# microsoft/foldingdiff

Hardware: AMD Instinct MI355X
Metric: backbones/sec (L=128, T=1000, bs=512) (higher is better)
Workload: dtype f32 (fp16 hi/lo split operands, 3x v_mfma_f32_{32x32x16,16x16x32}_f16 per product, fp32 accumulate)

## Files before the change

### foldingdiff_amd/csrc/ffn16.hip

```cpp
#include <cstdlib>
#include <type_traits>

#include "fdmi_kernels.h"
#include "img_common.h"

namespace fdmi {
namespace ffn {

typedef float f32x4 __attribute__((ext_vector_type(4)));
typedef const __attribute__((address_space(3))) u32x4* lds_cu128_t;
__device__ __forceinline__ unsigned lds_addr(const void* p) { return (unsigned)(unsigned long long)(lds_ptr_t)(const_cast<void*>(p)); }
__device__ __forceinline__ u32x4 lds_u128(unsigned a) { return *(lds_cu128_t)(unsigned long long)a; }
__device__ __forceinline__ f16x8 lds_f16x8(unsigned a) { return __builtin_bit_cast(f16x8, lds_u128(a)); }

__device__ __forceinline__ void swap16(unsigned& vdst, unsigned& src) {
  const auto r = __builtin_amdgcn_permlane16_swap(vdst, src, false, false);
  vdst = r[0];
  src = r[1];
}
__device__ __forceinline__ float quad_sum(float x) {
  unsigned a = __builtin_bit_cast(unsigned, x), b = a;
  swap32(a, b);
  float m = __builtin_bit_cast(float, a) + __builtin_bit_cast(float, b);
  a = __builtin_bit_cast(unsigned, m);
  b = a;
  swap16(a, b);
  return __builtin_bit_cast(float, a) + __builtin_bit_cast(float, b);
}

template <int V> using IC = std::integral_constant<int, V>;
template <int LO, int HI, class F>
__device__ __forceinline__ void static_for(F&& f) {
  if constexpr (LO < HI) {
    f(IC<LO>{});
    static_for<LO + 1, HI>(f);
  }
}

#ifndef FDMI_FFN_DBG
#define FDMI_FFN_DBG 0
#endif
#ifndef FDMI_FFN_ST_AUX
#define FDMI_FFN_ST_AUX 0
#endif
#ifndef FDMI_FFN_PRIO
#define FDMI_FFN_PRIO 2
#endif

__device__ __forceinline__ f32x4 mfma16(const f16x8& a, const f16x8& b, const f32x4& c) {
  return __builtin_amdgcn_mfma_f32_16x16x32_f16(a, b, c, 0, 0, 0);
}

constexpr int NW = 8;
constexpr int TILE = 2048;
constexpr int STEP = 4 * TILE;
constexpr int SPS = 2;
constexpr int STAGE = SPS * STEP;
constexpr int NST = 3;
constexpr int PPW = STAGE / 1024 / NW;
constexpr int OFF_W = 0;
constexpr int OFF_X = NST * STAGE;
__host__ __device__ constexpr int off_p(int nkt) { return OFF_X + NW * nkt * 1024; }

template <int NKT, bool TAIL, bool PROF>
__global__ __launch_bounds__(64 * NW) void ffn16_kernel(FfnArgs p) {
  static_assert(NKT == 12 || NKT == 6, "d_model 384 or 192, intermediate size 2 d_model");
  constexpr int D = 32 * NKT;
  constexpr int NG = NKT;
  constexpr int SPG = 2 * NKT;
  constexpr int STG = SPG / SPS;
  static_assert(STG % NST == 0, "a group is a whole number of ring turns: its first stage always sits in slot 0");
  constexpr int NSA = TAIL ? NKT * NKT / 2 : 0;
  static_assert((NSA / SPS) % NST == 0 && NSA % SPS == 0, "whole ring turns");
  constexpr int W_BYTES = (NSA / SPS + NG * STG) * STAGE;
  constexpr int OFF_P = off_p(NKT);
  constexpr int OFF_P1 = OFF_P + 5 * D * 4;
  extern __shared__ __attribute__((aligned(16))) unsigned char smem[];
  const int tid = threadIdx.x, lane = tid & 63;
  const int wq = __builtin_amdgcn_readfirstlane(tid >> 6);
  const int grp = wq >> 2;
  unsigned smem0 = __builtin_amdgcn_readfirstlane(lds_addr(smem));
  asm volatile("" : "+s"(smem0));
  auto lane_id = [&]() __attribute__((always_inline)) {
    int ln;
    asm volatile("v_mbcnt_lo_u32_b32 %0, -1, 0\n\tv_mbcnt_hi_u32_b32 %0, -1, %0" : "=v"(ln));
    return ln;
  };
  auto lane_off_of = [](int ln) __attribute__((always_inline)) { return (unsigned)((ln >> 4) * 256 + (ln & 15) * 16); };

  {
    float* par = reinterpret_cast<float*>(smem + OFF_P);
    for (int i = tid; i < 2 * D; i += 64 * NW) par[i] = p.bi[i];
    for (int i = tid; i < D; i += 64 * NW) {
      par[2 * D + i] = p.bd[i];
      par[3 * D + i] = p.gamma[i];
      par[4 * D + i] = p.beta[i] * p.out_scale;
      if constexpr (TAIL) {
        par[5 * D + i] = p.bo[i] * (1.0f / p.ao_scale);
        par[6 * D + i] = p.g1[i];
        par[7 * D + i] = p.b1[i] * p.a_scale;
      }
    }
  }

  int w_src = 0, w_slot = 0;
  const __amdgpu_buffer_rsrc_t rs_w = __builtin_amdgcn_make_buffer_rsrc(const_cast<unsigned char*>(p.wimg), 0, W_BYTES, 0x00020000);
  auto issue_w = [&]() __attribute__((always_inline)) {
    const lds_ptr_t dst = (lds_ptr_t)(unsigned long long)(smem0 + OFF_W + (unsigned)__builtin_amdgcn_readfirstlane(w_slot));
    const int so = __builtin_amdgcn_readfirstlane(w_src);
    const int vo = lane_id() * 16;
#pragma unroll
    for (int k = 0; k < PPW; ++k) dma16(rs_w, dst + (wq + NW * k) * 1024, vo, so + (wq + NW * k) * 1024);
    w_src = w_src + STAGE == W_BYTES ? 0 : w_src + STAGE;
    w_slot = w_slot + STAGE == NST * STAGE ? 0 : w_slot + STAGE;
  };

  f16x8 ah[NKT];
  const __amdgpu_buffer_rsrc_t rs_a =
      __builtin_amdgcn_make_buffer_rsrc(const_cast<unsigned char*>(TAIL ? p.cimg : p.aimg), 0, p.a_bytes, 0x00020000);
  const __amdgpu_buffer_rsrc_t rs_h = __builtin_amdgcn_make_buffer_rsrc(const_cast<unsigned char*>(TAIL ? p.hres : p.aimg), 0, p.a_bytes, 0x00020000);
  auto row_off = [&](int r0) __attribute__((always_inline)) {
    const int ln = lane_id();
    const int row = r0 + 16 * wq + (ln & 15);
    return (unsigned)(((row >> 5) * (NKT * 256) + (row & 31)) * 16 + (ln >> 4) * 512);
  };
  u32x4 tl[NKT];
  auto load_hi = [&](int r0) __attribute__((always_inline)) {
    const unsigned hoff = row_off(r0);
#pragma unroll
    for (int kt = 0; kt < NKT; ++kt)
      ah[kt] = __builtin_bit_cast(f16x8, __builtin_amdgcn_raw_buffer_load_b128(rs_a, (int)hoff, kt * 8 * 512, 0));
  };
  auto load_lo = [&](auto KT, unsigned hoff) __attribute__((always_inline)) {
    constexpr int kt = decltype(KT)::value;
    tl[kt] = __builtin_bit_cast(u32x4, __builtin_amdgcn_raw_buffer_load_b128(rs_a, (int)hoff, (kt * 8 + 4) * 512, 0));
  };
  auto commit_lo = [&]() __attribute__((always_inline)) {
    const unsigned ax = smem0 + OFF_X + (unsigned)(wq * NKT * 1024 + lane_id() * 16);
#pragma unroll
    for (int kt = 0; kt < NKT; ++kt) *(__attribute__((address_space(3))) u32x4*)(unsigned long long)(ax + (unsigned)(kt * 1024)) = tl[kt];
  };
  const __amdgpu_buffer_rsrc_t rs_o = __builtin_amdgcn_make_buffer_rsrc(p.out, 0, p.out_bytes, 0x00020000);
  auto load_res = [&](auto KT, unsigned hoff, f32x4 (&Yr)[2 * NKT]) __attribute__((always_inline)) {
    constexpr int kt = decltype(KT)::value;
    Yr[2 * kt] = __builtin_bit_cast(f32x4, __builtin_amdgcn_raw_buffer_load_b128(rs_h, (int)hoff, kt * 8 * 512, 0));
    Yr[2 * kt + 1] = __builtin_bit_cast(f32x4, __builtin_amdgcn_raw_buffer_load_b128(rs_h, (int)hoff, (kt * 8 + 4) * 512, 0));
  };

  const bool rec = PROF && blockIdx.x == 0 && p.stamps != nullptr;
  unsigned long long* stp = PROF ? p.stamps + (size_t)wq * 16 * 16 : nullptr;
  int slot = 0;
#define FD_STAMP(i) do { if (PROF) { if (rec && slot < 16 && lane == 0) stp[slot * 16 + (i)] = __builtin_amdgcn_s_memtime(); } } while (0)
#define FD_SB() __builtin_amdgcn_sched_barrier(0)
#define FD_STAMP_G(i) do { if (PROF) { if (rec && slot == 0 && G == 1 && lane == 0) stp[15 * 16 + (i)] = __builtin_amdgcn_s_memtime(); } } while (0)

  const int n_pass = p.dims ? min(p.panels, __builtin_amdgcn_readfirstlane(p.dims[1]) >> 7) : p.panels;
  if ((int)blockIdx.x >= n_pass) return;
  const float os_up = p.up_scale, os_dn = p.down_scale, hs = 0.5f * p.g_scale;
  const f32x4 zero4 = {0.f, 0.f, 0.f, 0.f};
  f32x4 Y[2 * NKT];
  f32x4 U[4];
  f32x4 Up[4];
  u32x4 uh[2], ul[2];

  load_hi((int)blockIdx.x * 128);
  {
    const unsigned hoff = row_off((int)blockIdx.x * 128);
    static_for<0, NKT>([&](auto KT) __attribute__((always_inline)) { load_lo(KT, hoff); });
    if constexpr (TAIL) static_for<0, NKT>([&](auto KT) __attribute__((always_inline)) { load_res(KT, hoff, Y); });
  }
  issue_w();
  issue_w();
  issue_w();
  FD_WAIT_VM(3 * PPW);
  commit_lo();
  FD_WAIT_VM(2 * PPW);
  barrier_keep_vm();

  auto gelu_piece = [&](auto P, unsigned abq) __attribute__((always_inline)) {
    constexpr int pc = decltype(P)::value, pr = pc >> 2, j = pc & 3;
    const u32x2 b = *(const __attribute__((address_space(3))) u32x2*)(unsigned long long)(abq + (unsigned)((32 * pr + 2 * j) * 4));
    float o0 = __builtin_fmaf(Up[2 * pr + (j >> 1)][2 * (j & 1)], os_up, __builtin_bit_cast(float, (unsigned)b[0]));
    float o1 = __builtin_fmaf(Up[2 * pr + (j >> 1)][2 * (j & 1) + 1], os_up, __builtin_bit_cast(float, (unsigned)b[1]));
#if !(FDMI_FFN_DBG & 1)
    const float h0 = o0 * hs, h1 = o1 * hs;
    o0 = __builtin_fmaf(h0, erf_rational(o0 * 0.70710678118654752440f), h0);
    o1 = __builtin_fmaf(h1, erf_rational(o1 * 0.70710678118654752440f), h1);
#endif
    unsigned a, c;
    split_pair(o0, o1, a, c);
    uh[pr][j] = a;
    ul[pr][j] = c;
  };

  auto steps = [&](auto S0, auto S1, auto GEL, unsigned abq) __attribute__((always_inline)) {
    constexpr int s0 = decltype(S0)::value, s1 = decltype(S1)::value;
    constexpr bool gel = decltype(GEL)::value == 1, pha = decltype(GEL)::value == 2;
    auto stage_top = [&]() __attribute__((always_inline)) {
      FD_WAIT_VM(PPW);
      barrier_keep_vm();
      issue_w();
    };
    f16x8 fx[4], fy[4], xl;
    unsigned a_W, a_X;
    {
      const int ln = lane_id();
      a_W = smem0 + OFF_W + lane_off_of(ln);
      a_X = smem0 + OFF_X + (unsigned)(wq * NKT * 1024 + ln * 16);
      asm volatile("" : "+v"(a_W), "+v"(a_X));
    }
    auto plane_reads = [&](auto S, auto LO, f16x8 (&f)[4]) __attribute__((always_inline)) {
      constexpr int s = decltype(S)::value, lo = decltype(LO)::value;
      constexpr unsigned off = (unsigned)(((s / SPS) % NST) * STAGE + (s % SPS) * STEP + lo * 1024);
#if FDMI_FFN_DBG & 8
      if constexpr (lo == 1) {
#pragma unroll
        for (int t = 0; t < 4; ++t) f[t] = fx[t];
      } else
#endif
#pragma unroll
      for (int t = 0; t < 4; ++t) f[t] = lds_f16x8(a_W + off + (unsigned)(t * TILE));
      if constexpr (pha) {
        if constexpr (lo == 0 && s % (NKT / 2) == 0) xl = lds_f16x8(a_X + (unsigned)((s / (NKT / 2)) * 1024));
      } else {
        if constexpr (lo == 0 && s < NKT) xl = lds_f16x8(a_X + (unsigned)(s * 1024));
      }
    };
    auto mm = [&](auto S, auto WHICH, const f16x8 (&f)[4]) __attribute__((always_inline)) {
      constexpr int s = decltype(S)::value, which = decltype(WHICH)::value;
      if constexpr (pha) {
        constexpr int kt = s / (NKT / 2), q = s % (NKT / 2);
#pragma unroll
        for (int t = 0; t < 4; ++t) Y[4 * q + t] = mfma16(f[t], which == 1 ? xl : ah[kt], Y[4 * q + t]);
      } else if constexpr (s < NKT) {
#if !(FDMI_FFN_DBG & 4)
#pragma unroll
        for (int t = 0; t < 4; ++t) U[t] = mfma16(f[t], which == 1 ? xl : ah[s], U[t]);
#endif
      } else {
#if !(FDMI_FFN_DBG & 2)
        constexpr int pr = (s - NKT) / (NKT / 2), q = (s - NKT) % (NKT / 2);
#pragma unroll
        for (int t = 0; t < 4; ++t) Y[4 * q + t] = mfma16(f[t], __builtin_bit_cast(f16x8, which == 1 ? ul[pr] : uh[pr]), Y[4 * q + t]);
#endif
      }
    };
    plane_reads(S0, IC<0>{}, fx);
    FD_SB();
    static_for<s0, s1>([&](auto S) __attribute__((always_inline)) {
      constexpr int s = decltype(S)::value;
      constexpr bool top = s % SPS == SPS - 1;
      plane_reads(S, IC<1>{}, fy);
      FD_SB();
      if constexpr (top) {
        if (grp == 0) stage_top();
      }
#if FDMI_FFN_PRIO
      __builtin_amdgcn_s_setprio(FDMI_FFN_PRIO);
#endif
      mm(S, IC<0>{}, fx);
      mm(S, IC<1>{}, fx);
#if FDMI_FFN_PRIO
      __builtin_amdgcn_s_setprio(0);
#endif
      FD_SB();
      if constexpr (top) {
        if (grp != 0) stage_top();
      }
      if constexpr (s + 1 < s1) plane_reads(IC<s + 1>{}, IC<0>{}, fx);
      FD_SB();
      if constexpr (gel) {
        if (grp == 0) {
          static_for<0, 8>([&](auto P) __attribute__((always_inline)) {
            if constexpr (1 + decltype(P)::value * (NKT - 2) / 8 == s) gelu_piece(P, abq);
          });
        }
        FD_SB();
      }
      mm(S, IC<2>{}, fy);
      FD_SB();
      if constexpr (gel) {
        if (grp != 0) {
          static_for<0, 8>([&](auto P) __attribute__((always_inline)) {
            if constexpr (1 + decltype(P)::value * (NKT - 2) / 8 == s) gelu_piece(P, abq);
          });
        }
        FD_SB();
      }
    });
  };

  for (int panel = blockIdx.x; panel < n_pass; panel += (int)gridDim.x) {
    FD_STAMP(0);
    if constexpr (TAIL) {
      const int ln = lane_id();
      const int g = ln >> 4;
      const unsigned pb1 = smem0 + OFF_P1 + (unsigned)(8 * g * 4);
      const unsigned ax = smem0 + OFF_X + (unsigned)(wq * NKT * 1024 + ln * 16);
      {
        const float c = p.hres_inv * (1.0f / p.ao_scale);
#pragma unroll
        for (int kt = 0; kt < NKT; ++kt) {
          const u32x4 rh = __builtin_bit_cast(u32x4, Y[2 * kt]), rl = __builtin_bit_cast(u32x4, Y[2 * kt + 1]);
          const u32x4 b0 = lds_u128(pb1 + (unsigned)(kt * 128)), b1 = lds_u128(pb1 + (unsigned)(kt * 128 + 16));
#pragma unroll
          for (int j = 0; j < 2; ++j)
#pragma unroll
            for (int e = 0; e < 4; e += 2) {
              const unsigned hw = rh[2 * j + e / 2], lw = rl[2 * j + e / 2];
              const unsigned bw0 = j == 0 ? b0[e] : b1[e], bw1 = j == 0 ? b0[e + 1] : b1[e + 1];
              float v0 = fma_mix_lo(hw, c, __builtin_bit_cast(float, bw0));
              float v1 = fma_mix_hi(hw, c, __builtin_bit_cast(float, bw1));
              Y[2 * kt + j][e] = fma_mix_lo(lw, c, v0);
              Y[2 * kt + j][e + 1] = fma_mix_hi(lw, c, v1);
            }
        }
      }
      steps(IC<0>{}, IC<NSA>{}, IC<2>{}, 0u);
      const float os_ao = p.ao_scale;
      float sum = 0.f;
#pragma unroll
      for (int t = 0; t < 2 * NKT; ++t)
#pragma unroll
        for (int e = 0; e < 4; ++e) {
          Y[t][e] *= os_ao;
          sum += Y[t][e];
        }
      const float inv_n = 1.0f / (float)D;
      float mean = quad_sum(sum) * inv_n;
      asm volatile("" : "+v"(mean));
      float t2 = 0.f;
#pragma unroll
      for (int t = 0; t < 2 * NKT; ++t)
#pragma unroll
        for (int e = 0; e < 4; ++e) {
          const float dl = Y[t][e] - mean;
          Y[t][e] = dl;
          t2 = __builtin_fmaf(dl, dl, t2);
        }
      const float rstd = (1.0f / sqrtf(__builtin_fmaf(quad_sum(t2), inv_n, p.eps1))) * p.a_scale;
#pragma unroll
      for (int kt = 0; kt < NKT; ++kt) {
        const u32x4 g0 = lds_u128(pb1 + (unsigned)(D * 4 + kt * 128)), g1 = lds_u128(pb1 + (unsigned)(D * 4 + kt * 128 + 16));
        const u32x4 e0 = lds_u128(pb1 + (unsigned)(2 * D * 4 + kt * 128)), e1 = lds_u128(pb1 + (unsigned)(2 * D * 4 + kt * 128 + 16));
        float o[8];
#pragma unroll
        for (int e = 0; e < 4; ++e) {
          o[e] = __builtin_fmaf(Y[2 * kt][e] * rstd, __builtin_bit_cast(float, (unsigned)g0[e]), __builtin_bit_cast(float, (unsigned)e0[e]));
          o[4 + e] = __builtin_fmaf(Y[2 * kt + 1][e] * rstd, __builtin_bit_cast(float, (unsigned)g1[e]), __builtin_bit_cast(float, (unsigned)e1[e]));
        }
        u32x4 hv, lv;
#pragma unroll
        for (int j = 0; j < 4; ++j) {
          unsigned a, b;
          split_pair(o[2 * j], o[2 * j + 1], a, b);
          hv[j] = a;
          lv[j] = b;
        }
        ah[kt] = __builtin_bit_cast(f16x8, hv);
        *(__attribute__((address_space(3))) u32x4*)(unsigned long long)(ax + (unsigned)(kt * 1024)) = lv;
      }
    }
#pragma unroll
    for (int t = 0; t < 2 * NKT; ++t) Y[t] = zero4;
#pragma unroll
    for (int t = 0; t < 4; ++t) U[t] = zero4;
    steps(IC<0>{}, IC<NKT>{}, IC<0>{}, 0u);
    for (int G = 0; G < NG; ++G) {
#pragma unroll
      for (int t = 0; t < 4; ++t) {
        Up[t] = U[t];
        U[t] = zero4;
      }
      unsigned abq = smem0 + OFF_P + (unsigned)((64 * G + 8 * (lane_id() >> 4)) * 4);
      asm volatile("" : "+v"(abq));
      FD_STAMP_G(0);
      FD_STAMP_G(1);
      if (G + 1 < NG) {
#ifdef FDMI_FFN_NOPIPE
        static_for<0, 8>([&](auto P) __attribute__((always_inline)) { gelu_piece(P, abq); });
        steps(IC<0>{}, IC<NKT>{}, IC<0>{}, abq);
#else
        steps(IC<0>{}, IC<NKT>{}, IC<1>{}, abq);
#endif
      } else {
        static_for<0, 8>([&](auto P) __attribute__((always_inline)) { gelu_piece(P, abq); });
      }
      FD_STAMP_G(2);
      steps(IC<NKT>{}, IC<SPG>{}, IC<0>{}, 0u);
      FD_STAMP_G(3);
      if (slot == 0) FD_STAMP(1 + (G < 12 ? G : 11));
    }
    {
      const int ln = lane_id();
      const int g = ln >> 4;
      const unsigned pb = smem0 + OFF_P + (unsigned)((2 * D + 8 * g) * 4);
      const unsigned ax = smem0 + OFF_X + (unsigned)(wq * NKT * 1024 + ln * 16);
      const float ri = p.resid_inv;
      float sum = 0.f;
#pragma unroll
      for (int kt = 0; kt < NKT; ++kt) {
        const u32x4 b0 = lds_u128(pb + (unsigned)(kt * 128)), b1 = lds_u128(pb + (unsigned)(kt * 128 + 16));
        const u32x4 rh = __builtin_bit_cast(u32x4, ah[kt]), rl = lds_u128(ax + (unsigned)(kt * 1024));
#pragma unroll
        for (int j = 0; j < 2; ++j)
#pragma unroll
          for (int e = 0; e < 4; e += 2) {
            const unsigned bw0 = j == 0 ? b0[e] : b1[e], bw1 = j == 0 ? b0[e + 1] : b1[e + 1];
            float v0 = __builtin_fmaf(Y[2 * kt + j][e], os_dn, __builtin_bit_cast(float, bw0));
            float v1 = __builtin_fmaf(Y[2 * kt + j][e + 1], os_dn, __builtin_bit_cast(float, bw1));
            const unsigned hw = rh[2 * j + e / 2], lw = rl[2 * j + e / 2];
            v0 = fma_mix_lo(hw, ri, v0);
            v1 = fma_mix_hi(hw, ri, v1);
            v0 = fma_mix_lo(lw, ri, v0);
            v1 = fma_mix_hi(lw, ri, v1);
            Y[2 * kt + j][e] = v0;
            Y[2 * kt + j][e + 1] = v1;
            sum += v0;
            sum += v1;
          }
      }
      const int next = panel + (int)gridDim.x;
      load_hi(next * 128);
      const unsigned noff = row_off(next * 128);
      const float inv_n = 1.0f / (float)D;
      float mean = quad_sum(sum) * inv_n;
      asm volatile("" : "+v"(mean));
      float t2 = 0.f;
#pragma unroll
      for (int t = 0; t < 2 * NKT; ++t)
#pragma unroll
        for (int e = 0; e < 4; ++e) {
          const float dl = Y[t][e] - mean;
          Y[t][e] = dl;
          t2 = __builtin_fmaf(dl, dl, t2);
        }
      const float rstd = (1.0f / sqrtf(__builtin_fmaf(quad_sum(t2), inv_n, p.eps))) * p.out_scale;
      const unsigned ooff = row_off(panel * 128);
      static_for<0, NKT>([&](auto KT) __attribute__((always_inline)) {
        constexpr int kt = decltype(KT)::value;
        const u32x4 g0 = lds_u128(pb + (unsigned)(D * 4 + kt * 128)), g1 = lds_u128(pb + (unsigned)(D * 4 + kt * 128 + 16));
        const u32x4 e0 = lds_u128(pb + (unsigned)(2 * D * 4 + kt * 128)), e1 = lds_u128(pb + (unsigned)(2 * D * 4 + kt * 128 + 16));
        float o[8];
#pragma unroll
        for (int e = 0; e < 4; ++e) {
          o[e] = __builtin_fmaf(Y[2 * kt][e] * rstd, __builtin_bit_cast(float, (unsigned)g0[e]), __builtin_bit_cast(float, (unsigned)e0[e]));
          o[4 + e] = __builtin_fmaf(Y[2 * kt + 1][e] * rstd, __builtin_bit_cast(float, (unsigned)g1[e]), __builtin_bit_cast(float, (unsigned)e1[e]));
        }
        u32x4 hv, lv;
#pragma unroll
        for (int j = 0; j < 4; ++j) {
          unsigned a, b;
          split_pair(o[2 * j], o[2 * j + 1], a, b);
          hv[j] = a;
          lv[j] = b;
        }
#if FDMI_FFN_DBG & 16
        if (hv[0] == 0x12345678u && lv[1] == 0x9abcdef0u)
#endif
        {
          __builtin_amdgcn_raw_buffer_store_b128(hv, rs_o, (int)ooff, kt * 8 * 512, FDMI_FFN_ST_AUX);
          __builtin_amdgcn_raw_buffer_store_b128(lv, rs_o, (int)ooff, (kt * 8 + 4) * 512, FDMI_FFN_ST_AUX);
        }
        load_lo(KT, noff);
        if constexpr (TAIL) load_res(KT, noff, Y);
        FD_SB();
      });
    }
    FD_STAMP(13);
    FD_WAIT_VM(0);
    commit_lo();
    FD_STAMP(14);
    ++slot;
  }
  FD_WAIT_VM(0);
#undef FD_STAMP
#undef FD_STAMP_G
#undef FD_SB
}

static int n_cu_of(int dev) {
  static int cached[64] = {0};
  if (dev < 0 || dev >= 64) return 256;
  if (cached[dev] == 0) {
    hipDeviceProp_t prop;
    cached[dev] = (hipGetDeviceProperties(&prop, dev) == hipSuccess && prop.multiProcessorCount > 0) ? prop.multiProcessorCount : 256;
  }
  return cached[dev];
}

template <int NKT, bool TAIL>
static bool launch(const FfnArgs& p, hipStream_t s) {
  constexpr int SMEM = off_p(NKT) + (TAIL ? 8 : 5) * 32 * NKT * 4;
  static int attr_state[64] = {0};
  int dev = 0;
  (void)hipGetDevice(&dev);
  if (dev < 0 || dev >= 64) dev = 0;
  if (attr_state[dev] == 0) {
    bool ok = true;
    for (const void* f : {reinterpret_cast<const void*>(&ffn16_kernel<NKT, TAIL, false>), reinterpret_cast<const void*>(&ffn16_kernel<NKT, TAIL, true>)})
      ok = ok && hipFuncSetAttribute(f, hipFuncAttributeMaxDynamicSharedMemorySize, SMEM) == hipSuccess;
    attr_state[dev] = ok ? 1 : -1;
  }
  if (attr_state[dev] < 0) return false;
  int grid = n_cu_of(dev);
  if (grid > p.panels) grid = p.panels;
  if (grid <= 0) return true;
  if (p.stamps) hipLaunchKernelGGL((ffn16_kernel<NKT, TAIL, true>), dim3(grid), dim3(64 * NW), SMEM, s, p);
  else hipLaunchKernelGGL((ffn16_kernel<NKT, TAIL, false>), dim3(grid), dim3(64 * NW), SMEM, s, p);
  return hipGetLastError() == hipSuccess;
}

}

bool ffn16_supported(int d_model, int d_ff) { return (d_model == 384 || d_model == 192) && d_ff == 2 * d_model; }

bool launch_ffn16(const FfnArgs& p, int d_model, hipStream_t s) {
  if (p.cimg) return d_model == 384 ? ffn::launch<12, true>(p, s) : ffn::launch<6, true>(p, s);
  return d_model == 384 ? ffn::launch<12, false>(p, s) : ffn::launch<6, false>(p, s);
}

}
```

Before: 82.10.

## Split LDS operand reads into halves and carry prefetch across step phases

Restructures the inner MFMA step loop so weight-plane LDS reads are issued in two-tile halves interleaved with half-width MFMA groups, and the next step's reads are prefetched earlier. The fragment registers now live outside the step lambda so prefetched operands carry across phase boundaries (up->down, down->up, layernorm->up), controlled by a CARRY bitmask. Stage-top barrier placement is made configurable. The aim is to hide LDS latency behind MFMAs at step and phase transitions, at the cost of higher register pressure and more complex scheduling.

```diff
diff --git a/foldingdiff_amd/csrc/ffn16.hip b/foldingdiff_amd/csrc/ffn16.hip
--- a/foldingdiff_amd/csrc/ffn16.hip
+++ b/foldingdiff_amd/csrc/ffn16.hip
@@ -45,6 +45,15 @@
 #endif
 #ifndef FDMI_FFN_PRIO
 #define FDMI_FFN_PRIO 2
+#endif
+#ifndef FDMI_FFN_CARRY
+#define FDMI_FFN_CARRY 5
+#endif
+#ifndef FDMI_FFN_TOP0
+#define FDMI_FFN_TOP0 1
+#endif
+#ifndef FDMI_FFN_TOP1
+#define FDMI_FFN_TOP1 2
 #endif
 
 __device__ __forceinline__ f32x4 mfma16(const f16x8& a, const f16x8& b, const f32x4& c) {
@@ -193,15 +202,20 @@
     ul[pr][j] = c;
   };
 
-  auto steps = [&](auto S0, auto S1, auto GEL, unsigned abq) __attribute__((always_inline)) {
+  f16x8 fx[4], fy[4], xl;
+  bool more = true;
+  auto steps_c = [&](auto S0, auto S1, auto GEL, unsigned abq, auto CIN, auto COUT) __attribute__((always_inline)) {
     constexpr int s0 = decltype(S0)::value, s1 = decltype(S1)::value;
     constexpr bool gel = decltype(GEL)::value == 1, pha = decltype(GEL)::value == 2;
+    constexpr bool cin = decltype(CIN)::value != 0;
+    constexpr int cout = decltype(COUT)::value;
     auto stage_top = [&]() __attribute__((always_inline)) {
       FD_WAIT_VM(PPW);
       barrier_keep_vm();
+#if !(FDMI_FFN_DBG & 32)
       issue_w();
+#endif
     };
-    f16x8 fx[4], fy[4], xl;
     unsigned a_W, a_X;
     {
       const int ln = lane_id();
@@ -209,65 +223,103 @@
       a_X = smem0 + OFF_X + (unsigned)(wq * NKT * 1024 + ln * 16);
       asm volatile("" : "+v"(a_W), "+v"(a_X));
     }
-    auto plane_reads = [&](auto S, auto LO, f16x8 (&f)[4]) __attribute__((always_inline)) {
-      constexpr int s = decltype(S)::value, lo = decltype(LO)::value;
+    auto plane_reads = [&](auto S, auto LO, auto T0, f16x8 (&f)[4]) __attribute__((always_inline)) {
+      constexpr int s = decltype(S)::value, lo = decltype(LO)::value, t0 = decltype(T0)::value;
       constexpr unsigned off = (unsigned)(((s / SPS) % NST) * STAGE + (s % SPS) * STEP + lo * 1024);
 #if FDMI_FFN_DBG & 8
       if constexpr (lo == 1) {
 #pragma unroll
-        for (int t = 0; t < 4; ++t) f[t] = fx[t];
+        for (int t = t0; t < t0 + 2; ++t) f[t] = fx[t];
       } else
 #endif
 #pragma unroll
-      for (int t = 0; t < 4; ++t) f[t] = lds_f16x8(a_W + off + (unsigned)(t * TILE));
-      if constexpr (pha) {
-        if constexpr (lo == 0 && s % (NKT / 2) == 0) xl = lds_f16x8(a_X + (unsigned)((s / (NKT / 2)) * 1024));
+      for (int t = t0; t < t0 + 2; ++t) f[t] = lds_f16x8(a_W + off + (unsigned)(t * TILE));
+    };
+    auto xl_read = [&](auto S) __attribute__((always_inline)) {
+      constexpr int s = decltype(S)::value;
+      if constexpr (s == s1) {
+        if constexpr (!pha && !gel) xl = lds_f16x8(a_X);
+      } else if constexpr (pha) {
+        if constexpr (s % (NKT / 2) == 0) xl = lds_f16x8(a_X + (unsigned)((s / (NKT / 2)) * 1024));
       } else {
-        if constexpr (lo == 0 && s < NKT) xl = lds_f16x8(a_X + (unsigned)(s * 1024));
+        if constexpr (s < NKT) xl = lds_f16x8(a_X + (unsigned)(s * 1024));
       }
     };
-    auto mm = [&](auto S, auto WHICH, const f16x8 (&f)[4]) __attribute__((always_inline)) {
-      constexpr int s = decltype(S)::value, which = decltype(WHICH)::value;
+    auto mm = [&](auto S, auto WHICH, auto T0, const f16x8 (&f)[4]) __attribute__((always_inline)) {
+      constexpr int s = decltype(S)::value, which = decltype(WHICH)::value, t0 = decltype(T0)::value;
       if constexpr (pha) {
         constexpr int kt = s / (NKT / 2), q = s % (NKT / 2);
 #pragma unroll
-        for (int t = 0; t < 4; ++t) Y[4 * q + t] = mfma16(f[t], which == 1 ? xl : ah[kt], Y[4 * q + t]);
+        for (int t = t0; t < t0 + 2; ++t) Y[4 * q + t] = mfma16(f[t], which == 1 ? xl : ah[kt], Y[4 * q + t]);
       } else if constexpr (s < NKT) {
 #if !(FDMI_FFN_DBG & 4)
 #pragma unroll
-        for (int t = 0; t < 4; ++t) U[t] = mfma16(f[t], which == 1 ? xl : ah[s], U[t]);
+        for (int t = t0; t < t0 + 2; ++t) U[t] = mfma16(f[t], which == 1 ? xl : ah[s], U[t]);
 #endif
       } else {
 #if !(FDMI_FFN_DBG & 2)
         constexpr int pr = (s - NKT) / (NKT / 2), q = (s - NKT) % (NKT / 2);
 #pragma unroll
-        for (int t = 0; t < 4; ++t) Y[4 * q + t] = mfma16(f[t], __builtin_bit_cast(f16x8, which == 1 ? ul[pr] : uh[pr]), Y[4 * q + t]);
+        for (int t = t0; t < t0 + 2; ++t) Y[4 * q + t] = mfma16(f[t], __builtin_bit_cast(f16x8, which == 1 ? ul[pr] : uh[pr]), Y[4 * q + t]);
 #endif
       }
     };
-    plane_reads(S0, IC<0>{}, fx);
+    auto prio = [&](int on) __attribute__((always_inline)) {
+#if FDMI_FFN_PRIO
+      if (on) __builtin_amdgcn_s_setprio(FDMI_FFN_PRIO);
+      else __builtin_amdgcn_s_setprio(0);
+#endif
+    };
+    if constexpr (!cin) {
+      plane_reads(S0, IC<0>{}, IC<0>{}, fx);
+      plane_reads(S0, IC<0>{}, IC<2>{}, fx);
+      xl_read(S0);
+      plane_reads(S0, IC<1>{}, IC<0>{}, fy);
+      plane_reads(S0, IC<1>{}, IC<2>{}, fy);
+    }
     FD_SB();
     static_for<s0, s1>([&](auto S) __attribute__((always_inline)) {
       constexpr int s = decltype(S)::value;
       constexpr bool top = s % SPS == SPS - 1;
-      plane_reads(S, IC<1>{}, fy);
+      constexpr bool last = s + 1 == s1;
+      auto ahead = [&](auto F) __attribute__((always_inline)) {
+        if constexpr (!last || cout == 1) F();
+        else if constexpr (cout == 2) {
+          if (more) F();
+        }
+      };
+      auto top_at = [&](auto POS) __attribute__((always_inline)) {
+        if constexpr (top) {
+          constexpr int pos = decltype(POS)::value;
+          if constexpr (pos == FDMI_FFN_TOP0) {
+            if (grp == 0) stage_top();
+            FD_SB();
+          }
+          if constexpr (pos == FDMI_FFN_TOP1) {
+            if (grp != 0) stage_top();
+            FD_SB();
+          }
+        }
+      };
+      top_at(IC<0>{});
+      prio(1);
+      mm(S, IC<0>{}, IC<0>{}, fx);
+      if constexpr (top && (FDMI_FFN_TOP0 == 1 || FDMI_FFN_TOP1 == 1)) {
+        prio(0);
+        FD_SB();
+        top_at(IC<1>{});
+        prio(1);
+      }
+      mm(S, IC<1>{}, IC<0>{}, fx);
+      prio(0);
       FD_SB();
-      if constexpr (top) {
-        if (grp == 0) stage_top();
-      }
-#if FDMI_FFN_PRIO
-      __builtin_amdgcn_s_setprio(FDMI_FFN_PRIO);
-#endif
-      mm(S, IC<0>{}, fx);
-      mm(S, IC<1>{}, fx);
-#if FDMI_FFN_PRIO
-      __builtin_amdgcn_s_setprio(0);
-#endif
+      top_at(IC<2>{});
+      ahead([&]() __attribute__((always_inline)) { plane_reads(IC<s + 1>{}, IC<0>{}, IC<0>{}, fx); });
       FD_SB();
-      if constexpr (top) {
-        if (grp != 0) stage_top();
-      }
-      if constexpr (s + 1 < s1) plane_reads(IC<s + 1>{}, IC<0>{}, fx);
+      prio(1);
+      mm(S, IC<0>{}, IC<2>{}, fx);
+      mm(S, IC<1>{}, IC<2>{}, fx);
+      prio(0);
       FD_SB();
       if constexpr (gel) {
         if (grp == 0) {
@@ -277,7 +329,13 @@
         }
         FD_SB();
       }
-      mm(S, IC<2>{}, fy);
+      ahead([&]() __attribute__((always_inline)) {
+        plane_reads(IC<s + 1>{}, IC<0>{}, IC<2>{}, fx);
+        xl_read(IC<s + 1>{});
+      });
+      FD_SB();
+      mm(S, IC<2>{}, IC<0>{}, fy);
+      mm(S, IC<2>{}, IC<2>{}, fy);
       FD_SB();
       if constexpr (gel) {
         if (grp != 0) {
@@ -287,7 +345,28 @@
         }
         FD_SB();
       }
+      ahead([&]() __attribute__((always_inline)) {
+        plane_reads(IC<s + 1>{}, IC<1>{}, IC<0>{}, fy);
+        plane_reads(IC<s + 1>{}, IC<1>{}, IC<2>{}, fy);
+      });
+      FD_SB();
     });
+  };
+  auto head_reads = [&]() __attribute__((always_inline)) {
+    unsigned a_W = smem0 + OFF_W + lane_off_of(lane_id());
+    asm volatile("" : "+v"(a_W));
+#pragma unroll
+    for (int t = 0; t < 4; ++t) fx[t] = lds_f16x8(a_W + (unsigned)(t * TILE));
+#pragma unroll
+    for (int t = 0; t < 4; ++t) fy[t] = lds_f16x8(a_W + (unsigned)(t * TILE + 1024));
+  };
+  auto steps = [&](auto S0, auto S1, auto GEL, unsigned abq) __attribute__((always_inline)) {
+    constexpr bool pha = decltype(GEL)::value == 2, up0 = decltype(GEL)::value == 0 && decltype(S0)::value == 0;
+    constexpr bool dn = decltype(S0)::value != 0, up1 = decltype(GEL)::value == 1;
+    constexpr bool c_ud = FDMI_FFN_CARRY & 1, c_du = FDMI_FFN_CARRY & 2, c_ln = (FDMI_FFN_CARRY & 4) && TAIL;
+    constexpr bool cin = dn ? c_ud : up1 ? c_du : up0 ? c_ln : false;
+    constexpr int cout = dn ? (c_du ? 2 : 0) : up1 ? (c_ud ? 1 : 0) : up0 ? (c_du ? 1 : 0) : (c_ln ? 1 : 0);
+    steps_c(S0, S1, GEL, abq, IC<cin ? 1 : 0>{}, IC<cout>{});
   };
 
   for (int panel = blockIdx.x; panel < n_pass; panel += (int)gridDim.x) {
@@ -359,6 +438,7 @@
         }
         ah[kt] = __builtin_bit_cast(f16x8, hv);
         *(__attribute__((address_space(3))) u32x4*)(unsigned long long)(ax + (unsigned)(kt * 1024)) = lv;
+        if (kt == 0) xl = __builtin_bit_cast(f16x8, lv);
       }
     }
 #pragma unroll
@@ -379,14 +459,20 @@
       if (G + 1 < NG) {
 #ifdef FDMI_FFN_NOPIPE
         static_for<0, 8>([&](auto P) __attribute__((always_inline)) { gelu_piece(P, abq); });
-        steps(IC<0>{}, IC<NKT>{}, IC<0>{}, abq);
+        steps_c(IC<0>{}, IC<NKT>{}, IC<0>{}, abq, IC<(FDMI_FFN_CARRY & 2) ? 1 : 0>{}, IC<(FDMI_FFN_CARRY & 1) ? 1 : 0>{});
 #else
         steps(IC<0>{}, IC<NKT>{}, IC<1>{}, abq);
 #endif
       } else {
-        static_for<0, 8>([&](auto P) __attribute__((always_inline)) { gelu_piece(P, abq); });
+        if constexpr (FDMI_FFN_CARRY & 1) head_reads();
+        FD_SB();
+        static_for<0, 8>([&](auto P) __attribute__((always_inline)) {
+          gelu_piece(P, abq);
+          FD_SB();
+        });
       }
       FD_STAMP_G(2);
+      more = G + 2 < NG;
       steps(IC<NKT>{}, IC<SPG>{}, IC<0>{}, 0u);
       FD_STAMP_G(3);
       if (slot == 0) FD_STAMP(1 + (G < 12 ? G : 11));
```

Result: no change. 82.42, median of 6 (+0.4%).
